# stevewongv/Sparse2Dense

Measured on AMD Instinct MI355X. Metric: LiDAR frames/sec (fwd+bwd), 150k-pt 0.1m-voxel synthetic Waymo scene, higher is better.
Workload: dtype bf16 (sparse stack: bf16 storage; dense neck/head: bf16 NHWC activations; fp32 accumulate, statistics, master weights, optimizer)

## Files before the change

include/s2d.h:

```cpp
#ifndef S2D_H_
#define S2D_H_

#include <stddef.h>
#include <stdint.h>

#ifdef __cplusplus
extern "C" {
#endif

typedef void *s2d_stream_t;

#define S2D_OK 0
#define S2D_ERR_INVALID_ARG (-1)
#define S2D_ERR_UNSUPPORTED (-2)
#define S2D_ERR_CAPACITY (-3)
#define S2D_ERR_WORKSPACE (-4)
#define S2D_ERR_COMM (-5)

int s2d_version(void);
int s2d_last_error(char *buf, size_t buf_len);
int s2d_build_info(char *buf, size_t buf_len);

size_t s2d_voxelize_batch_workspace_bytes(int frames, const int64_t *point_offsets, int max_points, int max_voxels);
int s2d_voxelize_batch_run(const float *points, int frames, const int64_t *point_offsets, int ndim,
// ... 473 lines not shown

#define S2D_ANCHOR_PREDICT_MAX_TASKS 8
typedef struct s2d_anchor_predict_task {
    const float *box_preds, *cls_preds, *dir_cls_preds, *anchors;
    int64_t num_anchors;
    int classes;
    int label_base;
} s2d_anchor_predict_task;
int s2d_anchor_predict_score(const s2d_anchor_predict_task *tasks, int num_tasks, int samples, int64_t max_anchors,
                             float score_threshold, float *score, int32_t *label, int32_t *count, s2d_stream_t stream);
int s2d_anchor_predict_boxes(const s2d_anchor_predict_task *tasks, int num_tasks, int samples, int64_t max_anchors,
                             const float *range6, const int64_t *order, const float *score_sorted, const int32_t *label,
                             const int32_t *offsets, const int32_t *counts, int max_count, int64_t total, float *boxes, float *scores,
                             int32_t *labels, int32_t *dir_labels, uint8_t *in_range, s2d_stream_t stream);
int s2d_anchor_predict_finish(const s2d_anchor_predict_task *tasks, int num_tasks, int samples, const float *boxes, const float *scores,
                              const int32_t *labels, const int32_t *dir_labels, const uint8_t *in_range, const int32_t *offsets,
                              const int32_t *counts, int64_t total, const int64_t *keep, const int32_t *n_keep, int max_keep,
                              int use_direction, float direction_offset, float *out_boxes, float *out_scores,
                              int64_t *out_labels, int32_t *out_count, s2d_stream_t stream);
int s2d_anchor_predict_finish_static(const s2d_anchor_predict_task *tasks, int num_tasks, int samples, const float *boxes,
                                     const float *scores, const int32_t *labels, const int32_t *dir_labels, const uint8_t *in_range,
                                     const int32_t *offsets, const int32_t *counts, int64_t total, const int64_t *keep,
                                     const int32_t *n_keep, int max_keep, int use_direction, float direction_offset, float *out_boxes,
                                     float *out_scores, int64_t *out_labels, int32_t *out_counts, s2d_stream_t stream);

int s2d_adam_max_tensors(void);
int s2d_adam_step_f32(int count, float *const *params, const float *const *grads, float *const *exp_avg,
                      float *const *exp_avg_sq, const int64_t *numel, float lr, float beta1, float beta2,
                      float eps, float weight_decay, int step, const float *clip_coef, s2d_stream_t stream);
size_t s2d_grad_norm_workspace_floats(int count, const int64_t *numel);
int s2d_grad_sumsq_f32(int count, const float *const *grads, const int64_t *numel, float *partial,
                       int *written, s2d_stream_t stream);
int s2d_grad_norm_finalize_f32(const float *partial, int n, float max_norm, float *out2, s2d_stream_t stream);

int s2d_comm_load_library(const char *path);
int s2d_comm_available(void);
int s2d_comm_unique_id(void *id128);
int s2d_comm_init(const void *id128, int nranks, int rank);
int s2d_comm_ranks(void);
int s2d_comm_shutdown(void);
int s2d_comm_allreduce_sum_f32(float *buf, int64_t count, s2d_stream_t stream);

int s2d_conv2d_pack_batch_bf16(int n, const float *const *weights, const int32_t *cin, const int32_t *cout, const int32_t *taps,
                               const int32_t *weight_nhwc, const int32_t *transpose_flip, void *const *packed_fwd, void *const *packed_dgrad,
                               s2d_stream_t stream);

int s2d_convt3d_mfma_fwd_stats_y16(const float *in, const void *packed, const float *bias, int batch, int cin, int cout, int d, int h, int w,
                                   void *out_bf16, float *stats_partial, s2d_stream_t stream);
int s2d_pointwise_conv_wgrad_norm_x16(const void *in_bf16, const float *in_scale_shift, const float *dout, int batch, int cin, int cout,
                                      int64_t positions, float *dweight, float *dbias, void *ws, size_t ws_bytes, s2d_stream_t stream);
int s2d_pcr_level_site_cache(void *buf, size_t bytes);
int s2d_pcr_level_fwd_y16_z16(const void *y, const float *bn_scale_shift, const float *head_params, const float *w2, const float *b2,
                              const int32_t *coors, const float *feats, int64_t m, int batch, int c, int co, int d, int h, int w, void *z_bf16,
                              float *z_stats, float *out8, void *ws, size_t ws_bytes, s2d_stream_t stream);
int s2d_pcr_level_bwd_sums_y16_z16(const void *y, const float *bn_scale_shift, const float *head_params, const int32_t *coors, const float *feats,
                                   int64_t m, int batch, int c, int d, int h, int w, const float *fwd_out8, const float *go_mask,
                                   const float *go_offset, const void *dz_bf16, const float *w2, int co, float *grads, float *bn_sums, void *ws,
                                   size_t ws_bytes, s2d_stream_t stream);
int s2d_pcr_level_bwd_apply_y16_d16_z16(const void *y, const float *bn_scale_shift, const float *head_params, const int32_t *coors,
                                        const float *feats, int64_t m, int batch, int c, int d, int h, int w, const float *fwd_out8,
                                        const float *go_mask, const float *go_offset, const void *dz_bf16, const float *w2, int co,
                                        const float *abd, void *dy_bf16, s2d_stream_t stream);
int s2d_pointwise_conv_wgrad_norm_x16_d16(const void *in_bf16, const float *in_scale_shift, const void *dout_bf16, int batch, int cin, int cout,
                                          int64_t positions, float *dweight, float *dbias, void *ws, size_t ws_bytes, s2d_stream_t stream);
int s2d_convt3d_mfma_x16_supported(int cin, int cout, int d, int h, int w);
int s2d_convt3d_mfma_fwd_stats_y16_norm_x16(const void *in_bf16, const float *in_scale_shift, const void *packed, const float *bias, int batch,
// ... 188 lines not shown
```

sparse2dense_amd/_lib.py:

```python
import ctypes
import os

_HERE = os.path.dirname(os.path.abspath(__file__))
LIB_PATH = os.path.join(_HERE, "lib", "libs2d_hip.so")

c_i32p = ctypes.c_void_p
c_f32p = ctypes.c_void_p
_I3 = ctypes.c_int32 * 3
_PFN_GEO = [ctypes.c_int64, ctypes.c_int, ctypes.c_int, ctypes.c_float, ctypes.c_float, ctypes.c_float, ctypes.c_float]
_F3 = ctypes.c_float * 3
_F6 = ctypes.c_float * 6


class CenterTask(ctypes.Structure):
    _fields_ = [(n, ctypes.c_void_p) for n in ("hm_logit", "reg", "height", "dim", "vel", "rot", "hm", "ind", "mask", "cat", "anno_box", "p",
                                               "d_logit", "d_reg", "d_height", "d_dim", "d_vel", "d_rot")] + [("classes", ctypes.c_int)]

class CenterPredictTask(ctypes.Structure):
    _fields_ = [("map", ctypes.c_void_p * 6), ("channel_stride", ctypes.c_int64 * 6), ("pixel_stride", ctypes.c_int64 * 6),
                ("classes", ctypes.c_int), ("label_base", ctypes.c_int)]


class AnchorPredictTask(ctypes.Structure):
    _fields_ = [(n, ctypes.c_void_p) for n in ("box_preds", "cls_preds", "dir_cls_preds", "anchors")] + \
# ... 228 lines not shown
                                    [c_f32p, c_f32p, c_f32p, c_f32p, c_f32p, ctypes.c_int, c_f32p, c_f32p, ctypes.c_void_p]),
    "s2d_pcr_level_bwd_apply_y16": (ctypes.c_int, [c_f32p, c_f32p, c_f32p, c_i32p, c_f32p, ctypes.c_int64] + [ctypes.c_int] * 5 +
                                    [c_f32p, c_f32p, c_f32p, c_f32p, c_f32p, ctypes.c_int, c_f32p, c_f32p, ctypes.c_void_p]),
    "s2d_pcr_level_bwd_apply_y16_d16": (ctypes.c_int, [c_f32p, c_f32p, c_f32p, c_i32p, c_f32p, ctypes.c_int64] + [ctypes.c_int] * 5 +
                                    [c_f32p, c_f32p, c_f32p, c_f32p, c_f32p, ctypes.c_int, c_f32p, c_f32p, ctypes.c_void_p]),
    "s2d_bev_iou_f32": (ctypes.c_int, [c_f32p, ctypes.c_int, c_f32p, ctypes.c_int, c_f32p, ctypes.c_void_p]),
    "s2d_nms_workspace_bytes": (ctypes.c_size_t, [ctypes.c_int]),
    "s2d_nms_rotated_bev": (ctypes.c_int, [c_f32p, ctypes.c_int, ctypes.c_float, ctypes.c_int, ctypes.c_void_p, ctypes.c_void_p, ctypes.c_void_p,
                                           ctypes.c_size_t, ctypes.c_void_p]),
    "s2d_nms_circle": (ctypes.c_int, [c_f32p, ctypes.c_int, ctypes.c_float, ctypes.c_int, ctypes.c_void_p, ctypes.c_void_p, ctypes.c_void_p,
                                      ctypes.c_size_t, ctypes.c_void_p]),
    "s2d_center_predict_score": (ctypes.c_int, [ctypes.c_void_p] + [ctypes.c_int] * 5 + [ctypes.c_float, ctypes.c_void_p] + [ctypes.c_float] * 5 +
                                 [ctypes.c_void_p] * 4),
    "s2d_center_predict_boxes": (ctypes.c_int, [ctypes.c_void_p] + [ctypes.c_int] * 5 + [ctypes.c_float] * 5 + [ctypes.c_void_p] * 5 +
                                 [ctypes.c_int, ctypes.c_int64] + [ctypes.c_void_p] * 4),
    "s2d_nms_batched_workspace_bytes": (ctypes.c_size_t, [ctypes.c_int64, ctypes.c_int]),
    "s2d_nms_rotated_bev_batched": (ctypes.c_int, [c_f32p, ctypes.c_int, c_i32p, c_i32p, ctypes.c_int, ctypes.c_int, ctypes.c_int64, ctypes.c_float,
                                                   ctypes.c_int, ctypes.c_void_p, ctypes.c_void_p, ctypes.c_void_p, ctypes.c_size_t, ctypes.c_void_p]),
    "s2d_nms_circle_batched": (ctypes.c_int, [c_f32p, ctypes.c_int, c_i32p, c_i32p, ctypes.c_int, ctypes.c_int, ctypes.c_int64, c_f32p,
                                              ctypes.c_int, ctypes.c_void_p, ctypes.c_void_p, ctypes.c_void_p, ctypes.c_size_t, ctypes.c_void_p]),
    "s2d_segment_topk": (ctypes.c_int, [ctypes.c_void_p, ctypes.c_int, ctypes.c_int64, ctypes.c_int64, ctypes.c_int, ctypes.c_void_p, ctypes.c_void_p,
                                        ctypes.c_void_p, ctypes.c_int64] + [ctypes.c_void_p] * 4),
    "s2d_predict_static_gather": (ctypes.c_int, [ctypes.c_void_p] * 6 + [ctypes.c_int] * 4 + [ctypes.c_int64] + [ctypes.c_void_p] * 5),
    "s2d_assign_label": (ctypes.c_int, [c_f32p, c_i32p, ctypes.c_int, ctypes.c_int, ctypes.c_float * 2, ctypes.c_float * 2] + [ctypes.c_int] * 5 +
                         [ctypes.c_double, ctypes.c_int] + [ctypes.c_void_p] * 7),
    "s2d_assign_label_tasks": (ctypes.c_int, [c_f32p, c_i32p, ctypes.c_int, ctypes.c_int, ctypes.POINTER(ctypes.c_int32), ctypes.c_int,
                                              ctypes.c_float * 2, ctypes.c_float * 2] + [ctypes.c_int] * 4 + [ctypes.c_double, ctypes.c_int] +
                               [ctypes.c_void_p] * 7),
    "s2d_adam_max_tensors": (ctypes.c_int, []),
    "s2d_adam_step_f32": (ctypes.c_int, [ctypes.c_int] + [ctypes.c_void_p] * 5 + [ctypes.c_float] * 5 + [ctypes.c_int, c_f32p, ctypes.c_void_p]),
    "s2d_grad_norm_workspace_floats": (ctypes.c_size_t, [ctypes.c_int, ctypes.c_void_p]),
    "s2d_grad_sumsq_f32": (ctypes.c_int, [ctypes.c_int, ctypes.c_void_p, ctypes.c_void_p, c_f32p, ctypes.c_void_p, ctypes.c_void_p]),
    "s2d_grad_norm_finalize_f32": (ctypes.c_int, [c_f32p, ctypes.c_int, ctypes.c_float, c_f32p, ctypes.c_void_p]),
    "s2d_dwconv7_supported": (ctypes.c_int, [ctypes.c_int]),
    "s2d_dwconv7_nhwc_bf16": (ctypes.c_int, [ctypes.c_void_p, c_f32p, c_f32p] + [ctypes.c_int] * 5 + [ctypes.c_void_p, ctypes.c_void_p]),
    "s2d_dwconv7_wgrad_workspace_bytes": (ctypes.c_size_t, [ctypes.c_int] * 4),
    "s2d_dwconv7_wgrad_nhwc_bf16": (ctypes.c_int, [ctypes.c_void_p, ctypes.c_void_p] + [ctypes.c_int] * 4 +
                                    [c_f32p, c_f32p, ctypes.c_void_p, ctypes.c_size_t, ctypes.c_void_p]),
    "s2d_comm_allreduce_sum_f32": (ctypes.c_int, [ctypes.c_void_p, ctypes.c_int64, ctypes.c_void_p]),
    "s2d_conv2d3x3_supported": (ctypes.c_int, [ctypes.c_int, ctypes.c_int]),
    "s2d_conv2d3x3_stats_tiles": (ctypes.c_int64, [ctypes.c_int] * 7),
    "s2d_conv2d3x3_pack_weights_bf16": (ctypes.c_int, [c_f32p, ctypes.c_int, ctypes.c_int, ctypes.c_int, ctypes.c_int,
                                                       ctypes.c_void_p, ctypes.c_void_p]),
    "s2d_conv2d3x3_tile_rows": (ctypes.c_int, [ctypes.c_int] * 7),
    "s2d_conv2d3x3_nhwc_bf16": (ctypes.c_int, [ctypes.c_void_p, ctypes.c_void_p, c_f32p, ctypes.c_void_p] +
                                [ctypes.c_int] * 7 + [ctypes.c_void_p, c_f32p, ctypes.c_void_p]),
    "s2d_bn_partials_finalize_f32": (ctypes.c_int, [c_f32p, ctypes.c_int, ctypes.c_int64, ctypes.c_int, c_f32p, c_f32p,
                                                    ctypes.c_float, ctypes.c_float, c_f32p, c_f32p, c_f32p, c_f32p, c_f32p, c_f32p,
                                                    ctypes.c_void_p, ctypes.c_void_p]),
    "s2d_bn_partials_finalize_ws_f32": (ctypes.c_int, [c_f32p, ctypes.c_int, ctypes.c_int64, ctypes.c_int, c_f32p, c_f32p,
                                                       ctypes.c_float, ctypes.c_float, c_f32p, c_f32p, c_f32p, c_f32p, c_f32p, c_f32p,
                                                       ctypes.c_void_p, ctypes.c_void_p, ctypes.c_size_t, ctypes.c_void_p]),
    "s2d_conv2d3x3_bnbwd_supported": (ctypes.c_int, [ctypes.c_int] * 4),
    "s2d_conv2d3x3_nhwc_bf16_bnbwd": (ctypes.c_int, [ctypes.c_void_p] * 3 + [ctypes.c_int] * 6 + [ctypes.c_void_p, ctypes.c_void_p, c_f32p, c_f32p,
                                                                                                    ctypes.c_int, c_f32p, ctypes.c_void_p]),
    "s2d_conv2d_debug_force": (ctypes.c_int, [ctypes.c_int] * 4),
    "s2d_conv2d_plan": (ctypes.c_int, [ctypes.c_int] * 9 + [ctypes.POINTER(ctypes.c_int32)]),
    "s2d_conv2d_wgrad_debug_force": (ctypes.c_int, [ctypes.c_int] * 2),
    "s2d_conv2d_wgrad_plan": (ctypes.c_int, [ctypes.c_int] * 8 + [ctypes.POINTER(ctypes.c_int32)]),
    "s2d_conv2d1x1_bnbwd_supported": (ctypes.c_int, [ctypes.c_int] * 2),
    "s2d_conv2d1x1_nhwc_bf16_bnbwd": (ctypes.c_int, [ctypes.c_void_p] * 3 + [ctypes.c_int] * 5 + [ctypes.c_void_p, ctypes.c_void_p, c_f32p, c_f32p,
                                                                                                    ctypes.c_int, c_f32p, ctypes.c_void_p]),
    "s2d_bn_partials_bwd_finalize_ws_f32": (ctypes.c_int, [c_f32p, ctypes.c_int, ctypes.c_int64, ctypes.c_int, c_f32p, c_f32p, c_f32p, c_f32p,
                                                           c_f32p, c_f32p, c_f32p, c_f32p, ctypes.c_void_p, ctypes.c_size_t, ctypes.c_void_p]),
    "s2d_bn_partials_sum_f32": (ctypes.c_int, [c_f32p, ctypes.c_int, ctypes.c_int64, ctypes.c_int, c_f32p, ctypes.c_int,
                                               ctypes.c_void_p]),
# ... 257 lines not shown
```

sparse2dense_amd/csrc/center_loss.hip:

```cpp
#include "s2d_common.h"

namespace s2d {

constexpr int FOCAL_BLOCKS = 256;

__device__ __forceinline__ float block_sum_256(float v, float *sh) {
#pragma unroll
    for (int d = 32; d >= 1; d >>= 1) v += __shfl_xor(v, d, 64);
    const int lane = threadIdx.x & 63, wid = threadIdx.x >> 6;
    __syncthreads();
    if (lane == 0) sh[wid] = v;
    __syncthreads();
    return (sh[0] + sh[1]) + (sh[2] + sh[3]);
}

__global__ __launch_bounds__(256) void focal_neg_kernel(const float *__restrict__ out, const float *__restrict__ target, int64_t n,
                                                        float *__restrict__ partial) {
    __shared__ float sh[4];
    float s = 0.f;
    for (int64_t i = (int64_t)blockIdx.x * 256 + threadIdx.x; i < n; i += (int64_t)gridDim.x * 256) {
        const float p = out[i], t = 1.f - target[i];
        const float t2 = t * t;
        s += logf(1.f - p) * p * p * (t2 * t2);
    }
// ... 21 lines not shown
        res[0] = -(pos + neg) / fmaxf(cnt, 1.f);
        res[1] = pos;
        res[2] = neg;
        res[3] = cnt;
    }
}

__global__ __launch_bounds__(256) void focal_bwd_neg_kernel(const float *__restrict__ out, const float *__restrict__ target, int64_t n,
                                                            const float *__restrict__ res, const float *__restrict__ go, float *__restrict__ dout) {
    const float coef = -go[0] / fmaxf(res[3], 1.f);
    for (int64_t i = (int64_t)blockIdx.x * 256 + threadIdx.x; i < n; i += (int64_t)gridDim.x * 256) {
        const float p = out[i], t = 1.f - target[i];
        const float t2 = t * t, q = 1.f - p;
        dout[i] = coef * (t2 * t2) * (2.f * p * logf(q) - p * p / q);
    }
}

__global__ __launch_bounds__(256) void focal_bwd_pos_kernel(const float *__restrict__ out, const int64_t *__restrict__ ind, const uint8_t *__restrict__ mask,
                                                            const int64_t *__restrict__ cat, int batch, int classes, int64_t hw, int max_objs,
                                                            const float *__restrict__ res, const float *__restrict__ go, float *__restrict__ dout) {
    const int i = blockIdx.x * 256 + threadIdx.x;
    if (i >= batch * max_objs || !mask[i]) return;
    const int b = i / max_objs;
    const int64_t at = ((int64_t)b * classes + cat[i]) * hw + ind[i];
    const float p = out[at], q = 1.f - p;
    const float coef = -go[0] / fmaxf(res[3], 1.f);
    atomicAdd(dout + at, coef * (q * q / p - 2.f * q * logf(p)));
}

__global__ __launch_bounds__(256) void regloss_fwd_kernel(const float *__restrict__ feat, const int64_t *__restrict__ ind, const uint8_t *__restrict__ mask,
                                                          const float *__restrict__ target, int batch, int channels, int64_t hw, int max_objs,
                                                          float *__restrict__ res) {
    __shared__ float sh[4];
    float cnt = 0.f;
    for (int i = threadIdx.x; i < batch * max_objs; i += 256) cnt += mask[i] ? 1.f : 0.f;
    cnt = block_sum_256(cnt, sh) + 1e-4f;
    for (int c = 0; c < channels; ++c) {
        float s = 0.f;
        for (int i = threadIdx.x; i < batch * max_objs; i += 256) {
            if (!mask[i]) continue;
            const int b = i / max_objs;
            s += fabsf(feat[((int64_t)b * channels + c) * hw + ind[i]] - target[(int64_t)i * channels + c]);
        }
        s = block_sum_256(s, sh);
        if (threadIdx.x == 0) res[c] = s / cnt;
    }
    if (threadIdx.x == 0) res[channels] = cnt;
}

__global__ __launch_bounds__(256) void regloss_bwd_kernel(const float *__restrict__ feat, const int64_t *__restrict__ ind, const uint8_t *__restrict__ mask,
                                                          const float *__restrict__ target, int batch, int channels, int64_t hw, int max_objs,
                                                          const float *__restrict__ res, const float *__restrict__ go, float *__restrict__ dfeat) {
    const int t = blockIdx.x * 256 + threadIdx.x;
    if (t >= batch * max_objs * channels) return;
    const int c = t % channels, i = t / channels;
    if (!mask[i]) return;
    const int b = i / max_objs;
    const int64_t at = ((int64_t)b * channels + c) * hw + ind[i];
    const float d = feat[at] - target[(int64_t)i * channels + c];
    const float sgn = d > 0.f ? 1.f : (d < 0.f ? -1.f : 0.f);
    atomicAdd(dfeat + at, go[c] * sgn / res[channels]);
}

constexpr int CT_MAX_TASKS = 8;
constexpr int CT_BLOCKS = 64;
constexpr int CT_RES = 16;
constexpr float CT_LO = 1e-4f, CT_HI = (float)(1 - 1e-4);

struct CtTable {
    s2d_center_task t[CT_MAX_TASKS];
};

__device__ __forceinline__ float ct_sigmoid(float x) { return 1.f / (1.f + expf(-x)); }

__device__ __forceinline__ int64_t ct_channel(const s2d_center_task &t, int c, int b, int64_t hw, int64_t cell, const float **map, float **dmap,
                                              int *tcol) {
    const bool vel = t.vel != nullptr;
    int cc, n;
    if (c < 2) { *map = t.reg; *dmap = t.d_reg; cc = c; n = 2; }
    else if (c == 2) { *map = t.height; *dmap = t.d_height; cc = 0; n = 1; }
// ... 150 lines not shown
                             int classes, int64_t hw, int max_objs, float *res, void *ws, size_t ws_bytes, s2d_stream_t stream) {
    S2D_CHECK_ARG(out && target && ind && mask && cat && res && batch > 0 && classes > 0 && hw > 0 && max_objs > 0, "focal_fwd: bad argument");
    if (!ws || ws_bytes < s2d_focal_workspace_bytes()) {
        set_error("focal_fwd: workspace too small");
        return S2D_ERR_WORKSPACE;
    }
    hipStream_t st = (hipStream_t)stream;
    const int64_t n = (int64_t)batch * classes * hw;
    const int nb = (int)std::min<int64_t>(FOCAL_BLOCKS, ceil_div(n, 256));
    hipLaunchKernelGGL(focal_neg_kernel, dim3(nb), dim3(256), 0, st, out, target, n, (float *)ws);
    hipLaunchKernelGGL(focal_finalize_kernel, dim3(1), dim3(256), 0, st, out, ind, mask, cat, batch, classes, hw, max_objs, (const float *)ws, nb,
                       res);
    S2D_LAUNCH_CHECK();
    return S2D_OK;
}

extern "C" int s2d_focal_bwd(const float *out, const float *target, const int64_t *ind, const uint8_t *mask, const int64_t *cat, int batch,
                             int classes, int64_t hw, int max_objs, const float *res, const float *go, float *dout, s2d_stream_t stream) {
    S2D_CHECK_ARG(out && target && ind && mask && cat && res && go && dout && batch > 0 && classes > 0 && hw > 0 && max_objs > 0,
                  "focal_bwd: bad argument");
    hipStream_t st = (hipStream_t)stream;
    const int64_t n = (int64_t)batch * classes * hw;
    hipLaunchKernelGGL(focal_bwd_neg_kernel, dim3((unsigned)std::min<int64_t>(2048, ceil_div(n, 256))), dim3(256), 0, st, out, target, n, res, go,
                       dout);
    hipLaunchKernelGGL(focal_bwd_pos_kernel, dim3((unsigned)ceil_div(batch * max_objs, 256)), dim3(256), 0, st, out, ind, mask, cat, batch, classes,
                       hw, max_objs, res, go, dout);
    S2D_LAUNCH_CHECK();
    return S2D_OK;
}

extern "C" int s2d_regloss_fwd(const float *feat, const int64_t *ind, const uint8_t *mask, const float *target, int batch, int channels,
                               int64_t hw, int max_objs, float *res, s2d_stream_t stream) {
    S2D_CHECK_ARG(feat && ind && mask && target && res && batch > 0 && channels > 0 && hw > 0 && max_objs > 0, "regloss_fwd: bad argument");
    hipLaunchKernelGGL(regloss_fwd_kernel, dim3(1), dim3(256), 0, (hipStream_t)stream, feat, ind, mask, target, batch, channels, hw, max_objs, res);
    S2D_LAUNCH_CHECK();
    return S2D_OK;
}

extern "C" int s2d_regloss_bwd(const float *feat, const int64_t *ind, const uint8_t *mask, const float *target, int batch, int channels,
                               int64_t hw, int max_objs, const float *res, const float *go, float *dfeat, s2d_stream_t stream) {
    S2D_CHECK_ARG(feat && ind && mask && target && res && go && dfeat && batch > 0 && channels > 0 && hw > 0 && max_objs > 0,
                  "regloss_bwd: bad argument");
    hipStream_t st = (hipStream_t)stream;
    if (int rc = zero_async(dfeat, (size_t)batch * channels * hw * sizeof(float), st)) return rc;
    hipLaunchKernelGGL(regloss_bwd_kernel, dim3((unsigned)ceil_div(batch * max_objs * channels, 256)), dim3(256), 0, st, feat, ind, mask, target,
                       batch, channels, hw, max_objs, res, go, dfeat);
    S2D_LAUNCH_CHECK();
    return S2D_OK;
}

extern "C" size_t s2d_center_tasks_loss_workspace_bytes(void) { return (size_t)CT_MAX_TASKS * CT_BLOCKS * sizeof(float) + 256; }

extern "C" int s2d_center_tasks_loss_fwd(const s2d_center_task *tasks, int num_tasks, int batch, int64_t hw, int max_objs,
                                         const float *code_weights, float weight, float *loss, float *loc_loss, float *res, void *ws,
                                         size_t ws_bytes, s2d_stream_t stream) {
    CtTable tb;
    int channels;
    int64_t max_n;
    if (int rc = ct_check_table(tasks, num_tasks, batch, hw, max_objs, false, &tb, &channels, &max_n)) return rc;
    S2D_CHECK_ARG(code_weights && loss && loc_loss && res, "center_tasks_loss_fwd: null argument");
    if (!ws || ws_bytes < s2d_center_tasks_loss_workspace_bytes()) {
        set_error("center_tasks_loss_fwd: workspace too small");
        return S2D_ERR_WORKSPACE;
    }
    hipStream_t st = (hipStream_t)stream;
    const int nb = (int)std::min<int64_t>(CT_BLOCKS, ceil_div(max_n, 256));
    hipLaunchKernelGGL(center_tasks_neg_kernel, dim3(nb, num_tasks), dim3(256), 0, st, tb, batch, hw, (float *)ws);
// ... 32 lines not shown
```

sparse2dense_amd/csrc/optim.hip:

```cpp
#include "s2d_common.h"

namespace s2d {

constexpr int ADAM_MAX_TENSORS = 48;
constexpr int ADAM_CHUNK = 256 * 4 * 4;

struct AdamTable {
    float *p[ADAM_MAX_TENSORS];
    const float *g[ADAM_MAX_TENSORS];
    float *m[ADAM_MAX_TENSORS];
    float *v[ADAM_MAX_TENSORS];
    int64_t n[ADAM_MAX_TENSORS];
    int first_block[ADAM_MAX_TENSORS + 1];
    int count;
};

__global__ __launch_bounds__(256) void adam_step_kernel(AdamTable tb, float lr, float beta1, float beta2, float eps, float wd, float bc1,
                                                        float bc2_sqrt, const float *__restrict__ clip_coef) {
    int ti = 0;
    while (ti + 1 < tb.count && (int)blockIdx.x >= tb.first_block[ti + 1]) ++ti;
    const int64_t base = (int64_t)(blockIdx.x - tb.first_block[ti]) * ADAM_CHUNK;
    float *p = tb.p[ti], *m = tb.m[ti], *v = tb.v[ti];
    const float *g = tb.g[ti];
    const int64_t n = tb.n[ti];
// ... 27 lines not shown
                v[i + e] = ve;
                p[i + e] = p[i + e] * decay - step * me / (sqrtf(ve) / bc2_sqrt + eps);
            }
        }
    }
}

struct NormTable {
    const float *g[ADAM_MAX_TENSORS];
    int64_t n[ADAM_MAX_TENSORS];
    int first_block[ADAM_MAX_TENSORS + 1];
    int count;
};

__global__ __launch_bounds__(256) void grad_sumsq_kernel(NormTable tb, float *__restrict__ partial) {
    __shared__ float red[4];
    int ti = 0;
    while (ti + 1 < tb.count && (int)blockIdx.x >= tb.first_block[ti + 1]) ++ti;
    const int64_t base = (int64_t)(blockIdx.x - tb.first_block[ti]) * ADAM_CHUNK;
    const float *g = tb.g[ti];
    const int64_t n = tb.n[ti];
    float s = 0.f;
    for (int j = 0; j < 16; ++j) {
        const int64_t i = base + (int64_t)j * 256 + threadIdx.x;
        if (i < n) { const float x = g[i]; s += x * x; }
    }
#pragma unroll
    for (int off = 32; off > 0; off >>= 1) s += __shfl_down(s, off, 64);
    if ((threadIdx.x & 63) == 0) red[threadIdx.x >> 6] = s;
    __syncthreads();
    if (threadIdx.x == 0) partial[blockIdx.x] = (red[0] + red[1]) + (red[2] + red[3]);
}

__global__ __launch_bounds__(256) void grad_norm_finalize_kernel(const float *__restrict__ partial, int n, float max_norm, float *__restrict__ out) {
    __shared__ double red[256];
    double s = 0;
    for (int i = threadIdx.x; i < n; i += 256) s += partial[i];
    red[threadIdx.x] = s;
    __syncthreads();
    for (int off = 128; off > 0; off >>= 1) {
        if ((int)threadIdx.x < off) red[threadIdx.x] += red[threadIdx.x + off];
        __syncthreads();
    }
    if (threadIdx.x == 0) {
        const float norm = (float)sqrt(red[0]);
        out[0] = norm;
        const float c = max_norm / (norm + 1e-6f);
        out[1] = c < 1.f ? c : 1.f;
    }
}

}

using namespace s2d;

extern "C" int s2d_adam_max_tensors(void) { return ADAM_MAX_TENSORS; }

extern "C" int s2d_adam_step_f32(int count, float *const *params, const float *const *grads, float *const *exp_avg, float *const *exp_avg_sq,
                                 const int64_t *numel, float lr, float beta1, float beta2, float eps, float weight_decay, int step,
                                 const float *clip_coef, s2d_stream_t stream) {
    S2D_CHECK_ARG(count >= 0 && count <= ADAM_MAX_TENSORS && step >= 1, "adam_step: bad count / step");
    if (count == 0) return S2D_OK;
    S2D_CHECK_ARG(params && grads && exp_avg && exp_avg_sq && numel, "adam_step: null table");
    AdamTable tb;
    int blocks = 0;
    for (int i = 0; i < count; ++i) {
// ... 15 lines not shown
extern "C" size_t s2d_grad_norm_workspace_floats(int count, const int64_t *numel) {
    size_t blocks = 0;
    for (int i = 0; i < count; ++i) blocks += (size_t)ceil_div(numel[i], ADAM_CHUNK);
    return blocks + 8;
}

extern "C" int s2d_grad_sumsq_f32(int count, const float *const *grads, const int64_t *numel, float *partial, int *written, s2d_stream_t stream) {
    S2D_CHECK_ARG(count >= 0 && count <= ADAM_MAX_TENSORS && written, "grad_sumsq: bad count");
    *written = 0;
    if (count == 0) return S2D_OK;
    S2D_CHECK_ARG(grads && numel && partial, "grad_sumsq: null argument");
    NormTable tb;
    int blocks = 0;
    for (int i = 0; i < count; ++i) {
        tb.g[i] = grads[i]; tb.n[i] = numel[i];
        tb.first_block[i] = blocks;
        blocks += (int)ceil_div(numel[i], ADAM_CHUNK);
    }
    tb.first_block[count] = blocks;
    tb.count = count;
    *written = blocks;
    if (blocks == 0) return S2D_OK;
    hipLaunchKernelGGL(grad_sumsq_kernel, dim3(blocks), dim3(256), 0, (hipStream_t)stream, tb, partial);
    S2D_LAUNCH_CHECK();
    return S2D_OK;
}

extern "C" int s2d_grad_norm_finalize_f32(const float *partial, int n, float max_norm, float *out2, s2d_stream_t stream) {
    S2D_CHECK_ARG(partial && out2 && n >= 0, "grad_norm_finalize: bad argument");
    hipLaunchKernelGGL(grad_norm_finalize_kernel, dim3(1), dim3(256), 0, (hipStream_t)stream, partial, n, max_norm, out2);
    S2D_LAUNCH_CHECK();
    return S2D_OK;
}
```

sparse2dense_amd/solver.py:

```python
import ctypes
import math

import numpy as np
import torch


def _ws(nbytes, device):
    return torch.empty(int(nbytes), dtype=torch.uint8, device=device)


def annealing_cos(start, end, pct):
    return end + (start - end) / 2 * (math.cos(math.pi * pct) + 1)


class OneCycle:

    def __init__(self, optimizer, total_step, lr_max, moms, div_factor, pct_start):
        self.optimizer, self.total_step = optimizer, int(total_step)
        self.lr_max, self.moms, self.div_factor, self.pct_start = lr_max, tuple(moms), div_factor, pct_start
        low = lr_max / div_factor
        split = int(pct_start * total_step)
        self.lr_phases = [(0, split, lambda p: annealing_cos(low, lr_max, p)),
                          (split, self.total_step, lambda p: annealing_cos(lr_max, low / 1e4, p))]
        self.mom_phases = [(0, split, lambda p: annealing_cos(self.moms[0], self.moms[1], p)),
                           (split, self.total_step, lambda p: annealing_cos(self.moms[1], self.moms[0], p))]
        if optimizer is not None:
            optimizer.lr, optimizer.mom = low, self.moms[0]

    def values(self, step):
        lr = mom = None
        for start, end, f in self.lr_phases:
            if step >= start:
                lr = f((step - start) / (end - start))
        for start, end, f in self.mom_phases:
            if step >= start:
                mom = f((step - start) / (end - start))
        return lr, mom
# ... 129 lines not shown
        return self.clip_and_step(max_norm=float("inf"))

    def _step_torch(self, ps, max_norm):
        norm = torch.linalg.vector_norm(torch.stack([torch.linalg.vector_norm(p.grad.detach().double()) for p in ps]))
        coef = 1.0 if math.isinf(max_norm) else torch.clamp(max_norm / (norm + 1e-6), max=1.0)
        with torch.no_grad():
            for p in ps:
                st = self._state(p)
                st["step"] += 1
                g = p.grad * coef
                p.mul_(1 - self.lr * self.wd)
                st["exp_avg"].mul_(self.mom).add_(g, alpha=1 - self.mom)
                st["exp_avg_sq"].mul_(self.beta).addcmul_(g, g, value=1 - self.beta)
                bc1, bc2 = 1 - self.mom ** st["step"], 1 - self.beta ** st["step"]
                p.addcdiv_(st["exp_avg"], st["exp_avg_sq"].sqrt() / math.sqrt(bc2) + self.eps, value=-self.lr / bc1)
        return norm

    def _step_hip(self, ps, max_norm):
        from . import _lib
        from .dense2d import _stream
        lib = _lib.load()
        ids = tuple(map(id, ps)) + tuple(p.data_ptr() for p in ps)
        c = self._hip_cache if getattr(self, "_hip_cache", None) is not None and self._hip_cache["ids"] == ids else None
        if c is not None and any((st["exp_avg"].data_ptr(), st["exp_avg_sq"].data_ptr()) != mv for st, mv in zip(c["states"], c["moments"])):
            c = None
        cap = lib.s2d_adam_max_tensors()
        vp = lambda ptrs: (ctypes.c_void_p * len(ptrs))(*ptrs)
        if c is None:
            dense = lambda t: t.is_contiguous() or (t.dim() == 4 and t.is_contiguous(memory_format=torch.channels_last))
            assert all(p.dtype == torch.float32 and dense(p) for p in ps), "OneCycleAdam: dense fp32 parameters expected"
            states = [self._state(p) for p in ps]
            numel = [p.numel() for p in ps]
            c = dict(ids=ids, states=states, numel=numel, numel_all=(ctypes.c_int64 * len(ps))(*numel), strides=[p.stride() for p in ps],
                     moments=[(st["exp_avg"].data_ptr(), st["exp_avg_sq"].data_ptr()) for st in states], groups=None, group_steps=None,
                     norm_chunks=[(i, min(i + cap, len(ps)), (ctypes.c_int64 * (min(i + cap, len(ps)) - i))(*numel[i:i + cap]))
                                  for i in range(0, len(ps), cap)])
            c["ws_floats"] = lib.s2d_grad_norm_workspace_floats(len(ps), c["numel_all"])
            self._hip_cache = c
        states = c["states"]
        same = lambda g, p: all(sg == sp for sg, sp, n in zip(g.stride(), p.stride(), p.shape) if n > 1)
        f32, pstrides = torch.float32, c["strides"]
        grads, gptr = [], []
        for i, p in enumerate(ps):
            g = p.grad
            if g.dtype is not f32 or (g.stride() != pstrides[i] and not same(g, p)):
                g = torch.empty_like(p).copy_(g)
            grads.append(g)
            gptr.append(g.data_ptr())
        steps = []
        for st in states:
            st["step"] += 1
            steps.append(st["step"])
        if c["group_steps"] is None or any(s != t + 1 for s, t in zip(steps, c["group_steps"])):
            by_step = {}
            for k, s_ in enumerate(steps):
                by_step.setdefault(s_, []).append(k)
            groups = []
            for members in by_step.values():
                for i in range(0, len(members), cap):
                    ks = members[i:i + cap]
                    groups.append(dict(ks=ks, n=len(ks), p=vp([ps[k].data_ptr() for k in ks]), m=vp([c["moments"][k][0] for k in ks]),
                                       v=vp([c["moments"][k][1] for k in ks]), numel=(ctypes.c_int64 * len(ks))(*[c["numel"][k] for k in ks])))
            c["groups"] = groups
        c["group_steps"] = steps
        dev, stream = ps[0].device, _stream()
        clip = None
        if not math.isinf(max_norm):
            ws = _ws(4 * c["ws_floats"], dev)
            written = 0
            for lo, hi, numel_chunk in c["norm_chunks"]:
                w = ctypes.c_int(0)
                _lib.check(lib.s2d_grad_sumsq_f32(hi - lo, vp(gptr[lo:hi]), numel_chunk, ws.data_ptr() + 4 * written, ctypes.byref(w), stream),
                           "s2d_grad_sumsq_f32")
                written += w.value
            clip = torch.empty(2, dtype=torch.float32, device=dev)
            _lib.check(lib.s2d_grad_norm_finalize_f32(ws.data_ptr(), written, float(max_norm), clip.data_ptr(), stream),
                       "s2d_grad_norm_finalize_f32")
        self._clip = clip
        for g in c["groups"]:
            ks = g["ks"]
            _lib.check(lib.s2d_adam_step_f32(g["n"], g["p"], vp([gptr[k] for k in ks]), g["m"], g["v"], g["numel"], float(self.lr), float(self.mom),
                                             float(self.beta), float(self.eps), float(self.wd), int(steps[ks[0]]),
                                             None if clip is None else clip.data_ptr() + 4, stream), "s2d_adam_step_f32")
        from .dense2d import refresh_pack_cache
        refresh_pack_cache()
        return None if clip is None else clip[0]


def build_one_cycle_optimizer(model, optimizer_config=None):
    wd = 0.01 if optimizer_config is None else getattr(optimizer_config, "wd", optimizer_config.get("wd", 0.01)
                                                       if isinstance(optimizer_config, dict) else 0.01)
    return OneCycleAdam([p for p in model.parameters() if p.requires_grad], lr=3e-3, mom=0.9, beta=0.99, wd=wd, model=model)


def build_one_cycle_scheduler(optimizer, lr_config, total_steps):
    cfg = dict(lr_config)
    assert cfg.pop("type", "one_cycle") == "one_cycle"
    return OneCycle(optimizer, total_steps, cfg["lr_max"], cfg["moms"], cfg["div_factor"], cfg["pct_start"])
```

Baseline: 223.9.

## Replace capped-batch Adam and grad-norm launches with a segment-table kernel

Adds a device-resident segment table (prefix offsets plus per-tensor p/g/m/v pointers) so one Adam launch and one grad sum-of-squares launch cover every parameter tensor, instead of several launches of at most the tensor cap each. Tables are built on the host, copied asynchronously through pinned memory, and kept in a small LRU keyed by gradient pointers, with events guarding reuse. Separately, the regression-loss forward now launches one block per channel instead of looping over channels in a single block. The cost is a binary search per block, extra table bookkeeping, and a fallback path during graph capture.

```diff
diff --git a/include/s2d.h b/include/s2d.h
--- a/include/s2d.h
+++ b/include/s2d.h
@@ -529,6 +529,13 @@
 int s2d_grad_sumsq_f32(int count, const float *const *grads, const int64_t *numel, float *partial,
                        int *written, s2d_stream_t stream);
 int s2d_grad_norm_finalize_f32(const float *partial, int n, float max_norm, float *out2, s2d_stream_t stream);
+size_t s2d_optim_segments_bytes(int count);
+int s2d_optim_segments_fill(int count, float *const *params, const float *const *grads, float *const *exp_avg,
+                            float *const *exp_avg_sq, const int64_t *numel, void *table, size_t table_bytes,
+                            int64_t *chunks, int64_t *norm_blocks);
+int s2d_adam_step_segments_f32(const void *table, int count, int64_t chunks, float lr, float beta1, float beta2, float eps,
+                               float weight_decay, int step, const float *clip_coef, s2d_stream_t stream);
+int s2d_grad_sumsq_segments_f32(const void *table, int count, int64_t norm_blocks, float *partial, s2d_stream_t stream);
 
 int s2d_comm_load_library(const char *path);
 int s2d_comm_available(void);
diff --git a/sparse2dense_amd/_lib.py b/sparse2dense_amd/_lib.py
--- a/sparse2dense_amd/_lib.py
+++ b/sparse2dense_amd/_lib.py
@@ -284,6 +284,11 @@
     "s2d_grad_norm_workspace_floats": (ctypes.c_size_t, [ctypes.c_int, ctypes.c_void_p]),
     "s2d_grad_sumsq_f32": (ctypes.c_int, [ctypes.c_int, ctypes.c_void_p, ctypes.c_void_p, c_f32p, ctypes.c_void_p, ctypes.c_void_p]),
     "s2d_grad_norm_finalize_f32": (ctypes.c_int, [c_f32p, ctypes.c_int, ctypes.c_float, c_f32p, ctypes.c_void_p]),
+    "s2d_optim_segments_bytes": (ctypes.c_size_t, [ctypes.c_int]),
+    "s2d_optim_segments_fill": (ctypes.c_int, [ctypes.c_int] + [ctypes.c_void_p] * 6 + [ctypes.c_size_t, ctypes.c_void_p, ctypes.c_void_p]),
+    "s2d_adam_step_segments_f32": (ctypes.c_int, [ctypes.c_void_p, ctypes.c_int, ctypes.c_int64] + [ctypes.c_float] * 5
+                                   + [ctypes.c_int, c_f32p, ctypes.c_void_p]),
+    "s2d_grad_sumsq_segments_f32": (ctypes.c_int, [ctypes.c_void_p, ctypes.c_int, ctypes.c_int64, c_f32p, ctypes.c_void_p]),
     "s2d_dwconv7_supported": (ctypes.c_int, [ctypes.c_int]),
     "s2d_dwconv7_nhwc_bf16": (ctypes.c_int, [ctypes.c_void_p, c_f32p, c_f32p] + [ctypes.c_int] * 5 + [ctypes.c_void_p, ctypes.c_void_p]),
     "s2d_dwconv7_wgrad_workspace_bytes": (ctypes.c_size_t, [ctypes.c_int] * 4),
diff --git a/sparse2dense_amd/csrc/center_loss.hip b/sparse2dense_amd/csrc/center_loss.hip
--- a/sparse2dense_amd/csrc/center_loss.hip
+++ b/sparse2dense_amd/csrc/center_loss.hip
@@ -77,20 +77,20 @@
                                                           const float *__restrict__ target, int batch, int channels, int64_t hw, int max_objs,
                                                           float *__restrict__ res) {
     __shared__ float sh[4];
-    float cnt = 0.f;
-    for (int i = threadIdx.x; i < batch * max_objs; i += 256) cnt += mask[i] ? 1.f : 0.f;
+    const int c = blockIdx.x;
+    float cnt = 0.f, s = 0.f;
+    for (int i = threadIdx.x; i < batch * max_objs; i += 256) {
+        if (!mask[i]) continue;
+        cnt += 1.f;
+        const int b = i / max_objs;
+        s += fabsf(feat[((int64_t)b * channels + c) * hw + ind[i]] - target[(int64_t)i * channels + c]);
+    }
     cnt = block_sum_256(cnt, sh) + 1e-4f;
-    for (int c = 0; c < channels; ++c) {
-        float s = 0.f;
-        for (int i = threadIdx.x; i < batch * max_objs; i += 256) {
-            if (!mask[i]) continue;
-            const int b = i / max_objs;
-            s += fabsf(feat[((int64_t)b * channels + c) * hw + ind[i]] - target[(int64_t)i * channels + c]);
-        }
-        s = block_sum_256(s, sh);
-        if (threadIdx.x == 0) res[c] = s / cnt;
-    }
-    if (threadIdx.x == 0) res[channels] = cnt;
+    s = block_sum_256(s, sh);
+    if (threadIdx.x == 0) {
+        res[c] = s / cnt;
+        if (c == 0) res[channels] = cnt;
+    }
 }
 
 __global__ __launch_bounds__(256) void regloss_bwd_kernel(const float *__restrict__ feat, const int64_t *__restrict__ ind, const uint8_t *__restrict__ mask,
@@ -307,7 +307,7 @@
 extern "C" int s2d_regloss_fwd(const float *feat, const int64_t *ind, const uint8_t *mask, const float *target, int batch, int channels,
                                int64_t hw, int max_objs, float *res, s2d_stream_t stream) {
     S2D_CHECK_ARG(feat && ind && mask && target && res && batch > 0 && channels > 0 && hw > 0 && max_objs > 0, "regloss_fwd: bad argument");
-    hipLaunchKernelGGL(regloss_fwd_kernel, dim3(1), dim3(256), 0, (hipStream_t)stream, feat, ind, mask, target, batch, channels, hw, max_objs, res);
+    hipLaunchKernelGGL(regloss_fwd_kernel, dim3(channels), dim3(256), 0, (hipStream_t)stream, feat, ind, mask, target, batch, channels, hw, max_objs, res);
     S2D_LAUNCH_CHECK();
     return S2D_OK;
 }
diff --git a/sparse2dense_amd/csrc/optim.hip b/sparse2dense_amd/csrc/optim.hip
--- a/sparse2dense_amd/csrc/optim.hip
+++ b/sparse2dense_amd/csrc/optim.hip
@@ -83,6 +83,159 @@
     if (threadIdx.x == 0) partial[blockIdx.x] = (red[0] + red[1]) + (red[2] + red[3]);
 }
 
+constexpr int SEG_CHUNK = ADAM_CHUNK;
+
+struct SegView {
+    const int64_t *vstart, *bstart, *n;
+    float *const *p;
+    const float *const *g;
+    float *const *m, *const *v;
+    int count;
+};
+
+__host__ __device__ inline size_t seg_table_bytes(int count) { return 2 * sizeof(int64_t) * ((size_t)count + 1) + (size_t)count * (sizeof(int64_t) + 4 * sizeof(void *)); }
+
+static SegView seg_view(const void *table, int count) {
+    SegView tb;
+    const char *b = static_cast<const char *>(table);
+    tb.vstart = reinterpret_cast<const int64_t *>(b);
+    tb.bstart = tb.vstart + count + 1;
+    tb.n = tb.bstart + count + 1;
+    tb.p = reinterpret_cast<float *const *>(tb.n + count);
+    tb.g = reinterpret_cast<const float *const *>(tb.p + count);
+    tb.m = tb.p + 2 * (size_t)count;
+    tb.v = tb.m + count;
+    tb.count = count;
+    return tb;
+}
+
+__device__ __forceinline__ int seg_find(const int64_t *__restrict__ vstart, int count, int64_t pos) {
+    int lo = 0, hi = count - 1;
+    while (lo < hi) {
+        const int mid = (lo + hi + 1) >> 1;
+        if (vstart[mid] <= pos) lo = mid; else hi = mid - 1;
+    }
+    return lo;
+}
+
+struct AdamConst {
+    float beta1, beta2, eps, bc2_sqrt, cc, decay, step;
+};
+
+__device__ __forceinline__ void adam_quad(float4 &pp, float4 &mm, float4 &vv, const float4 &gg, const AdamConst &k) {
+    float *pf = &pp.x, *mf = &mm.x, *vf = &vv.x;
+    const float *gf = &gg.x;
+#pragma unroll
+    for (int e = 0; e < 4; ++e) {
+        const float ge = gf[e] * k.cc;
+        mf[e] = k.beta1 * mf[e] + (1.f - k.beta1) * ge;
+        vf[e] = k.beta2 * vf[e] + (1.f - k.beta2) * ge * ge;
+        pf[e] = pf[e] * k.decay - k.step * mf[e] / (sqrtf(vf[e]) / k.bc2_sqrt + k.eps);
+    }
+}
+
+__device__ __forceinline__ void adam_group(float *p, const float *g, float *m, float *v, int64_t i, int64_t n, bool aligned, const AdamConst &k) {
+    if (i + 3 < n && aligned) {
+        float4 pp = *reinterpret_cast<float4 *>(p + i), mm = *reinterpret_cast<float4 *>(m + i), vv = *reinterpret_cast<float4 *>(v + i);
+        const float4 gg = *reinterpret_cast<const float4 *>(g + i);
+        adam_quad(pp, mm, vv, gg, k);
+        *reinterpret_cast<float4 *>(p + i) = pp;
+        *reinterpret_cast<float4 *>(m + i) = mm;
+        *reinterpret_cast<float4 *>(v + i) = vv;
+    } else {
+        for (int e = 0; e < 4; ++e) {
+            if (i + e >= n) break;
+            const float ge = g[i + e] * k.cc;
+            const float me = k.beta1 * m[i + e] + (1.f - k.beta1) * ge;
+            const float ve = k.beta2 * v[i + e] + (1.f - k.beta2) * ge * ge;
+            m[i + e] = me;
+            v[i + e] = ve;
+            p[i + e] = p[i + e] * k.decay - k.step * me / (sqrtf(ve) / k.bc2_sqrt + k.eps);
+        }
+    }
+}
+
+__device__ __forceinline__ bool quad_aligned(const void *a, const void *b, const void *c, const void *d) {
+    return ((reinterpret_cast<uintptr_t>(a) | reinterpret_cast<uintptr_t>(b) | reinterpret_cast<uintptr_t>(c) | reinterpret_cast<uintptr_t>(d)) & 15) == 0;
+}
+
+__global__ __launch_bounds__(256) void adam_step_segments_kernel(SegView tb, float lr, float beta1, float beta2, float eps, float wd, float bc1,
+                                                                 float bc2_sqrt, const float *__restrict__ clip_coef) {
+    const int64_t c0 = (int64_t)blockIdx.x * SEG_CHUNK;
+    const int s0 = seg_find(tb.vstart, tb.count, c0);
+    AdamConst k;
+    k.beta1 = beta1; k.beta2 = beta2; k.eps = eps; k.bc2_sqrt = bc2_sqrt;
+    k.cc = clip_coef ? clip_coef[0] : 1.f;
+    k.decay = 1.f - lr * wd; k.step = lr / bc1;
+    if (tb.vstart[s0 + 1] >= c0 + SEG_CHUNK) {
+        float *p = tb.p[s0], *m = tb.m[s0], *v = tb.v[s0];
+        const float *g = tb.g[s0];
+        const int64_t n = tb.n[s0], base = c0 - tb.vstart[s0];
+        const bool aligned = quad_aligned(p, g, m, v);
+        if (aligned && base + SEG_CHUNK <= n) {
+            float4 pp[4], mm[4], vv[4], gg[4];
+#pragma unroll
+            for (int j = 0; j < 4; ++j) {
+                const int64_t i = base + ((int64_t)j * 256 + threadIdx.x) * 4;
+                pp[j] = *reinterpret_cast<float4 *>(p + i);
+                gg[j] = *reinterpret_cast<const float4 *>(g + i);
+                mm[j] = *reinterpret_cast<float4 *>(m + i);
+                vv[j] = *reinterpret_cast<float4 *>(v + i);
+            }
+#pragma unroll
+            for (int j = 0; j < 4; ++j) {
+                const int64_t i = base + ((int64_t)j * 256 + threadIdx.x) * 4;
+                adam_quad(pp[j], mm[j], vv[j], gg[j], k);
+                *reinterpret_cast<float4 *>(p + i) = pp[j];
+                *reinterpret_cast<float4 *>(m + i) = mm[j];
+                *reinterpret_cast<float4 *>(v + i) = vv[j];
+            }
+        } else {
+            for (int j = 0; j < 4; ++j) {
+                const int64_t i = base + ((int64_t)j * 256 + threadIdx.x) * 4;
+                if (i < n) adam_group(p, g, m, v, i, n, aligned, k);
+            }
+        }
+        return;
+    }
+    int s = s0;
+    for (int j = 0; j < 4; ++j) {
+        const int64_t pos = c0 + ((int64_t)j * 256 + threadIdx.x) * 4;
+        while (s + 1 < tb.count && tb.vstart[s + 1] <= pos) ++s;
+        const int64_t i = pos - tb.vstart[s], n = tb.n[s];
+        if (i >= n) continue;
+        float *p = tb.p[s], *m = tb.m[s], *v = tb.v[s];
+        const float *g = tb.g[s];
+        adam_group(p, g, m, v, i, n, quad_aligned(p, g, m, v), k);
+    }
+}
+
+__global__ __launch_bounds__(256) void grad_sumsq_segments_kernel(SegView tb, float *__restrict__ partial) {
+    __shared__ float red[4];
+    const int s0 = seg_find(tb.bstart, tb.count, blockIdx.x);
+    const int64_t base = ((int64_t)blockIdx.x - tb.bstart[s0]) * ADAM_CHUNK;
+    const float *__restrict__ g = tb.g[s0];
+    const int64_t n = tb.n[s0];
+    float s = 0.f;
+    if (base + ADAM_CHUNK <= n) {
+        float x[16];
+#pragma unroll
+        for (int j = 0; j < 16; ++j) x[j] = g[base + (int64_t)j * 256 + threadIdx.x];
+#pragma unroll
+        for (int j = 0; j < 16; ++j) s += x[j] * x[j];
+    } else {
+        for (int j = 0; j < 16; ++j) {
+            const int64_t i = base + (int64_t)j * 256 + threadIdx.x;
+            if (i < n) { const float x = g[i]; s += x * x; }
+        }
+    }
+#pragma unroll
+    for (int off = 32; off > 0; off >>= 1) s += __shfl_down(s, off, 64);
+    if ((threadIdx.x & 63) == 0) red[threadIdx.x >> 6] = s;
+    __syncthreads();
+    if (threadIdx.x == 0) partial[blockIdx.x] = (red[0] + red[1]) + (red[2] + red[3]);
+}
+
 __global__ __launch_bounds__(256) void grad_norm_finalize_kernel(const float *__restrict__ partial, int n, float max_norm, float *__restrict__ out) {
     __shared__ double red[256];
     double s = 0;
@@ -164,3 +317,46 @@
     S2D_LAUNCH_CHECK();
     return S2D_OK;
 }
+
+extern "C" size_t s2d_optim_segments_bytes(int count) { return count > 0 ? seg_table_bytes(count) : 0; }
+
+extern "C" int s2d_optim_segments_fill(int count, float *const *params, const float *const *grads, float *const *exp_avg, float *const *exp_avg_sq,
+                                       const int64_t *numel, void *table, size_t table_bytes, int64_t *chunks, int64_t *norm_blocks) {
+    S2D_CHECK_ARG(count > 0 && params && grads && exp_avg && exp_avg_sq && numel && table && chunks && norm_blocks, "optim_segments_fill: bad argument");
+    S2D_CHECK_ARG(table_bytes >= seg_table_bytes(count), "optim_segments_fill: table of %zu bytes, %zu needed", table_bytes, seg_table_bytes(count));
+    char *b = static_cast<char *>(table);
+    int64_t *vstart = reinterpret_cast<int64_t *>(b), *bstart = vstart + count + 1, *n = bstart + count + 1;
+    void **p = reinterpret_cast<void **>(n + count), **g = p + count, **m = g + count, **v = m + count;
+    int64_t at = 0, blocks = 0;
+    for (int i = 0; i < count; ++i) {
+        S2D_CHECK_ARG(params[i] && grads[i] && exp_avg[i] && exp_avg_sq[i] && numel[i] >= 0, "optim_segments_fill: null tensor %d", i);
+        vstart[i] = at; bstart[i] = blocks; n[i] = numel[i];
+        p[i] = params[i]; g[i] = const_cast<float *>(grads[i]); m[i] = exp_avg[i]; v[i] = exp_avg_sq[i];
+        at += (numel[i] + 3) / 4 * 4;
+        blocks += ceil_div(numel[i], ADAM_CHUNK);
+    }
+    vstart[count] = at; bstart[count] = blocks;
+    *chunks = ceil_div(at, SEG_CHUNK);
+    *norm_blocks = blocks;
+    S2D_CHECK_ARG(blocks <= 0x7fffffff, "optim_segments_fill: %lld blocks", (long long)blocks);
+    return S2D_OK;
+}
+
+extern "C" int s2d_adam_step_segments_f32(const void *table, int count, int64_t chunks, float lr, float beta1, float beta2, float eps,
+                                          float weight_decay, int step, const float *clip_coef, s2d_stream_t stream) {
+    S2D_CHECK_ARG(table && count > 0 && chunks >= 0 && chunks <= 0x7fffffff && step >= 1, "adam_step_segments: bad argument");
+    if (chunks == 0) return S2D_OK;
+    const float bc1 = 1.f - powf(beta1, (float)step), bc2 = 1.f - powf(beta2, (float)step);
+    hipLaunchKernelGGL(adam_step_segments_kernel, dim3((unsigned)chunks), dim3(256), 0, (hipStream_t)stream, seg_view(table, count), lr, beta1, beta2, eps,
+                       weight_decay, bc1, sqrtf(bc2), clip_coef);
+    S2D_LAUNCH_CHECK();
+    return S2D_OK;
+}
+
+extern "C" int s2d_grad_sumsq_segments_f32(const void *table, int count, int64_t blocks, float *partial, s2d_stream_t stream) {
+    S2D_CHECK_ARG(table && count > 0 && blocks >= 0 && blocks <= 0x7fffffff && partial, "grad_sumsq_segments: bad argument");
+    if (blocks == 0) return S2D_OK;
+    hipLaunchKernelGGL(grad_sumsq_segments_kernel, dim3((unsigned)blocks), dim3(256), 0, (hipStream_t)stream, seg_view(table, count), partial);
+    S2D_LAUNCH_CHECK();
+    return S2D_OK;
+}
diff --git a/sparse2dense_amd/solver.py b/sparse2dense_amd/solver.py
--- a/sparse2dense_amd/solver.py
+++ b/sparse2dense_amd/solver.py
@@ -3,6 +3,26 @@
 
 import numpy as np
 import torch
+
+
+_TABLES_KEPT = 8
+
+
+def _segment_table(lib, slot, p, g, m, v, numel, device):
+    from . import _lib
+    n = len(g)
+    nbytes = lib.s2d_optim_segments_bytes(n)
+    if slot is None:
+        slot = dict(host=torch.empty(nbytes, dtype=torch.uint8, pin_memory=True), dev=torch.empty(nbytes, dtype=torch.uint8, device=device),
+                    used=torch.cuda.Event())
+    else:
+        slot["used"].synchronize()
+    chunks, norm_blocks = ctypes.c_int64(0), ctypes.c_int64(0)
+    _lib.check(lib.s2d_optim_segments_fill(n, p, (ctypes.c_void_p * n)(*g), m, v, numel, slot["host"].data_ptr(), nbytes, ctypes.byref(chunks),
+                                           ctypes.byref(norm_blocks)), "s2d_optim_segments_fill")
+    slot["dev"].copy_(slot["host"], non_blocking=True)
+    slot.update(chunks=chunks.value, norm_blocks=norm_blocks.value, grads=g)
+    return slot
 
 
 def _ws(nbytes, device):
@@ -198,7 +218,7 @@
             states = [self._state(p) for p in ps]
             numel = [p.numel() for p in ps]
             c = dict(ids=ids, states=states, numel=numel, numel_all=(ctypes.c_int64 * len(ps))(*numel), strides=[p.stride() for p in ps],
-                     moments=[(st["exp_avg"].data_ptr(), st["exp_avg_sq"].data_ptr()) for st in states], groups=None, group_steps=None,
+                     moments=[(st["exp_avg"].data_ptr(), st["exp_avg_sq"].data_ptr()) for st in states], groups=None, group_steps=None, tables={},
                      norm_chunks=[(i, min(i + cap, len(ps)), (ctypes.c_int64 * (min(i + cap, len(ps)) - i))(*numel[i:i + cap]))
                                   for i in range(0, len(ps), cap)])
             c["ws_floats"] = lib.s2d_grad_norm_workspace_floats(len(ps), c["numel_all"])
@@ -223,31 +243,69 @@
                 by_step.setdefault(s_, []).append(k)
             groups = []
             for members in by_step.values():
+                batches = []
                 for i in range(0, len(members), cap):
                     ks = members[i:i + cap]
-                    groups.append(dict(ks=ks, n=len(ks), p=vp([ps[k].data_ptr() for k in ks]), m=vp([c["moments"][k][0] for k in ks]),
-                                       v=vp([c["moments"][k][1] for k in ks]), numel=(ctypes.c_int64 * len(ks))(*[c["numel"][k] for k in ks])))
-            c["groups"] = groups
+                    batches.append(dict(ks=ks, n=len(ks), p=vp([ps[k].data_ptr() for k in ks]), m=vp([c["moments"][k][0] for k in ks]),
+                                        v=vp([c["moments"][k][1] for k in ks]), numel=(ctypes.c_int64 * len(ks))(*[c["numel"][k] for k in ks])))
+                groups.append((members, batches))
+            c["groups"], c["tables"] = groups, {}
         c["group_steps"] = steps
         dev, stream = ps[0].device, _stream()
+        capturing = torch.cuda.is_current_stream_capturing()
+        tables = c["tables"]
+
+        def table(ks):
+            key = tuple(ks)
+            gkey = tuple(gptr) if len(ks) == len(ps) else tuple(gptr[k] for k in ks)
+            kept = tables.get(key)
+            if kept is None:
+                kept = tables[key] = dict(p=vp([ps[k].data_ptr() for k in ks]), m=vp([c["moments"][k][0] for k in ks]),
+                                          v=vp([c["moments"][k][1] for k in ks]), numel=(ctypes.c_int64 * len(ks))(*[c["numel"][k] for k in ks]), lru=[])
+            lru = kept["lru"]
+            for i, t in enumerate(lru):
+                if t["grads"] == gkey:
+                    if i:
+                        lru.insert(0, lru.pop(i))
+                    return t
+            if capturing:
+                return None
+            slot = lru.pop() if len(lru) >= _TABLES_KEPT else None
+            lru.insert(0, _segment_table(lib, slot, kept["p"], gkey, kept["m"], kept["v"], kept["numel"], dev))
+            return lru[0]
         clip = None
         if not math.isinf(max_norm):
             ws = _ws(4 * c["ws_floats"], dev)
-            written = 0
-            for lo, hi, numel_chunk in c["norm_chunks"]:
-                w = ctypes.c_int(0)
-                _lib.check(lib.s2d_grad_sumsq_f32(hi - lo, vp(gptr[lo:hi]), numel_chunk, ws.data_ptr() + 4 * written, ctypes.byref(w), stream),
-                           "s2d_grad_sumsq_f32")
-                written += w.value
+            t = table(range(len(ps)))
             clip = torch.empty(2, dtype=torch.float32, device=dev)
+            if t is not None:
+                written = t["norm_blocks"]
+                _lib.check(lib.s2d_grad_sumsq_segments_f32(t["dev"].data_ptr(), len(ps), written, ws.data_ptr(), stream), "s2d_grad_sumsq_segments_f32")
+                if len(c["groups"]) > 1 and not capturing:
+                    t["used"].record()
+            else:
+                written = 0
+                for lo, hi, numel_chunk in c["norm_chunks"]:
+                    w = ctypes.c_int(0)
+                    _lib.check(lib.s2d_grad_sumsq_f32(hi - lo, vp(gptr[lo:hi]), numel_chunk, ws.data_ptr() + 4 * written, ctypes.byref(w), stream),
+                               "s2d_grad_sumsq_f32")
+                    written += w.value
             _lib.check(lib.s2d_grad_norm_finalize_f32(ws.data_ptr(), written, float(max_norm), clip.data_ptr(), stream),
                        "s2d_grad_norm_finalize_f32")
         self._clip = clip
-        for g in c["groups"]:
-            ks = g["ks"]
-            _lib.check(lib.s2d_adam_step_f32(g["n"], g["p"], vp([gptr[k] for k in ks]), g["m"], g["v"], g["numel"], float(self.lr), float(self.mom),
-                                             float(self.beta), float(self.eps), float(self.wd), int(steps[ks[0]]),
-                                             None if clip is None else clip.data_ptr() + 4, stream), "s2d_adam_step_f32")
+        hyper = (float(self.lr), float(self.mom), float(self.beta), float(self.eps), float(self.wd))
+        clip_ptr = None if clip is None else clip.data_ptr() + 4
+        for ks, batches in c["groups"]:
+            t = table(ks)
+            if t is not None:
+                _lib.check(lib.s2d_adam_step_segments_f32(t["dev"].data_ptr(), len(ks), t["chunks"], *hyper, int(steps[ks[0]]), clip_ptr, stream),
+                           "s2d_adam_step_segments_f32")
+                if not capturing:
+                    t["used"].record()
+                continue
+            for g in batches:
+                _lib.check(lib.s2d_adam_step_f32(g["n"], g["p"], vp([gptr[k] for k in g["ks"]]), g["m"], g["v"], g["numel"], *hyper,
+                                                 int(steps[ks[0]]), clip_ptr, stream), "s2d_adam_step_f32")
         from .dense2d import refresh_pack_cache
         refresh_pack_cache()
         return None if clip is None else clip[0]
```

Result: slower. 216.3 (-3.4%).
